# NivekNey/polars-matmul

Measured on AMD Instinct MI355X. Metric: cosine top-k queries/sec, higher is better.
Workload: dtype f32

## Files before the change

polars-matmul_amd/csrc/pmm_kernels.hip:

```cpp
#include "pmm_device.h"

#include <algorithm>

#include <hip/hip_runtime.h>
#include <math.h>
#include <stdint.h>

#include <type_traits>

namespace pmm {

hipError_t launch_norms_f32(const float *a, int64_t rows, int64_t d, int64_t ld, int squared,
                            float *out, float *inv, hipStream_t s) {
  if (rows <= 0) return hipSuccess;
  const int64_t threads = rows * 8;
  const unsigned grid = (unsigned)((threads + 255) / 256);
  norms_kernel<float><<<grid, 256, 0, s>>>(a, rows, d, ld, squared, out, inv);
  return hipGetLastError();
}
hipError_t launch_norms_pair_f32(const float *q, int64_t m, int64_t ldq, float *qout, const float *c,
                                 int64_t n, int64_t ldc, float *cout, float *cinv, int64_t d, int squared,
                                 hipStream_t s, void *zero, size_t zero_bytes) {
  const unsigned gq = (unsigned)((m * 8 + 255) / 256), gc = (unsigned)((n * 8 + 255) / 256);
  if (zero_bytes % 16 != 0 || ((uintptr_t)zero & 15)) return hipErrorInvalidValue;
// ... 1695 lines not shown
  auto lds = [&](int nsp) { return lds_base + RQ * nsp * 8; };
  if (a.ns <= 256) prologue_kernel<4, METRIC, LDSK><<<grid, 256, lds(256), s>>>(a);
  else if (a.ns <= 512) prologue_kernel<8, METRIC, LDSK><<<grid, 256, lds(512), s>>>(a);
  else prologue_kernel<16, METRIC, LDSK><<<grid, 256, lds(1024), s>>>(a);
  return hipGetLastError();
}
template <int METRIC>
static hipError_t launch_prologue_t(const PrologueArgs &a, unsigned grid, hipStream_t s) {
  return a.lds_seed ? launch_prologue_t2<METRIC, 1>(a, grid, s) : launch_prologue_t2<METRIC, 0>(a, grid, s);
}

#ifndef PMM_SEED_MFMA_DEFAULT
#define PMM_SEED_MFMA_DEFAULT 1
#endif
hipError_t launch_seeded_prologue(const float *q, int64_t ldq, int m, const float *c, int64_t ldc, int64_t n,
                                  int d, int dp, int ns, int k, int metric, float *qn, float *cn, bool corpus_norms,
                                  unsigned long long *gthr, void *z0, size_t z0_bytes, void *z1, size_t z1_bytes,
                                  hipStream_t s) {
  if (m <= 0) return hipSuccess;
  if (ns > kSeedMaxNs || k > ns || ns > n || dp % 32 != 0 || dp > kSeedDotsMaxD || d > dp || ldq % 4 != 0 ||
      ldc % 4 != 0 || (((uintptr_t)q | (uintptr_t)c | (uintptr_t)z0 | (uintptr_t)z1) & 15) || z0_bytes % 16 ||
      z1_bytes % 16)
    return hipErrorInvalidValue;
  PrologueArgs a{};
  a.q = q;
  a.ldq = ldq;
  a.m = m;
  a.c = c;
  a.ldc = ldc;
  a.n = n;
  a.d = d;
  a.dp = dp;
  a.ns = ns;
  a.k = k;
  a.squared = metric == kMetricEuclidean;
  a.qn = qn;
  a.cn = cn;
  a.cinv = cn + n;
  a.gthr = gthr;
  a.z0 = (uint4 *)z0;
  a.z1 = (uint4 *)z1;
  a.z0n = (int64_t)(z0_bytes / 16);
  a.z1n = (int64_t)(z1_bytes / 16);
#ifdef PMM_LAB
  a.ablate = getenv("PMM_PROLOGUE_ABLATE") ? atoi(getenv("PMM_PROLOGUE_ABLATE")) : 0;
#endif
  const char *le = getenv("PMM_SEED_LDS");
  a.lds_seed = (ns <= 256 && dp <= seedk::kLdsMaxDp && le && atoi(le) == 1) ? 1 : 0;
  const bool xf = metric != kMetricDot;
  const char *me = getenv("PMM_SEED_MFMA");
  const bool mfma_ok = ns == seedm::NSM && dp <= seedm::kMaxDp && !a.lds_seed && n >= seedm::NSM;
  a.mfma_seed = (mfma_ok && (me ? atoi(me) != 0 : PMM_SEED_MFMA_DEFAULT != 0)) ? 1 : 0;
  if (a.mfma_seed) {
    a.sblocks = (unsigned)((m + seedm::RM - 1) / seedm::RM);
    constexpr int T = seedm::NT;
    a.qblocks = xf ? (unsigned)((m * 8 + T - 1) / T) : 0u;
    a.cblocks = (xf && corpus_norms) ? (unsigned)((n * 8 + T - 1) / T) : 0u;
    a.zblocks = (unsigned)std::max<int64_t>(1, std::min<int64_t>((a.z0n + a.z1n + T - 1) / T, 16));
    const unsigned grid = a.sblocks + a.qblocks + a.cblocks + a.zblocks;
    if (metric == kMetricCosine) return launch_prologue_mfma_t<kMetricCosine>(a, grid, s);
    if (metric == kMetricDot) return launch_prologue_mfma_t<kMetricDot>(a, grid, s);
    return launch_prologue_mfma_t<kMetricEuclidean>(a, grid, s);
  }
  a.sblocks = (unsigned)((m + seedk::RQ - 1) / seedk::RQ);
  unsigned grid;
  if (a.lds_seed) {
    a.qblocks = 0u;
    grid = std::max<unsigned>(a.sblocks, (xf && corpus_norms) ? (unsigned)((n + 63) / 64) : 1u);
    a.cper = (n + grid - 1) / grid;
    a.cblocks = (xf && corpus_norms) ? 1u : 0u;
    a.zblocks = 0u;
  } else {
    a.qblocks = xf ? (unsigned)((m * 8 + 255) / 256) : 0u;
    a.cblocks = (xf && corpus_norms) ? (unsigned)((n * 8 + 255) / 256) : 0u;
    a.zblocks = (unsigned)std::max<int64_t>(1, std::min<int64_t>((a.z0n + a.z1n + 255) / 256, 64));
    grid = a.sblocks + a.qblocks + a.cblocks + a.zblocks;
  }
  if (metric == kMetricCosine) return launch_prologue_t<kMetricCosine>(a, grid, s);
  if (metric == kMetricDot) return launch_prologue_t<kMetricDot>(a, grid, s);
  return launch_prologue_t<kMetricEuclidean>(a, grid, s);
}

constexpr int kMergeRankMaxRows = 16384;
hipError_t launch_merge(const MergeArgs &a0, int loader, hipStream_t s) {
  if (a0.M <= 0) return hipSuccess;
  MergeArgs a = a0;
  static const int rank_env = getenv("PMM_MERGE_RANK") ? atoi(getenv("PMM_MERGE_RANK")) : -1;
  a.no_rank = rank_env == 0 || (rank_env < 0 && a.M > kMergeRankMaxRows);
  a.flags = getenv("PMM_MERGE_FLAGS") ? atoi(getenv("PMM_MERGE_FLAGS"))
                                     : (kMergeReverse | kMergePipelined | kMergeSplitRow);
  const bool sorted = loader == 1 && a.sorted && a.S <= 64 && a.k_out <= 256 && a.P <= 512 &&
                      !(getenv("PMM_MERGE_SORTED") && atoi(getenv("PMM_MERGE_SORTED")) == 0);
  static const int kp = getenv("PMM_KWAY_P") ? atoi(getenv("PMM_KWAY_P")) : 24;
  if (sorted && a.S >= 5 && a.S <= 8 && a.k_out <= 8 * (kp == 32 ? 32 : 24) &&
      !(getenv("PMM_MERGE_KWAY") && atoi(getenv("PMM_MERGE_KWAY")) == 0) &&
      (size_t)MPN(a.P) * 8 <= (size_t)64 * (kp == 32 ? 32 : 24) * 8) {
    static const int wpb = getenv("PMM_KWAY_WPB") ? atoi(getenv("PMM_KWAY_WPB")) : 4;
    const int rows_per_block = 8 * wpb;
    const unsigned grid = (unsigned)((a.M + rows_per_block - 1) / rows_per_block);
    if (kp != 32) {
      if (wpb == 4) (void)hipFuncSetAttribute((const void *)kway_merge_kernel<24>, hipFuncAttributeMaxDynamicSharedMemorySize, 160 * 1024);
      kway_merge_kernel<24><<<grid, 64 * wpb, (size_t)wpb * 64 * 24 * 8, s>>>(a);
    } else {
      if (wpb == 4) (void)hipFuncSetAttribute((const void *)kway_merge_kernel<32>, hipFuncAttributeMaxDynamicSharedMemorySize, 160 * 1024);
      kway_merge_kernel<32><<<grid, 64 * wpb, (size_t)wpb * 64 * 32 * 8, s>>>(a);
    }
    return hipGetLastError();
  }
  if (!(a.S >= 8 && a.k_out <= 64 && a.P <= 512 && !a.no_rank && a.ablate == 0) || sorted) a.flags &= ~kMergeSplitRow;
  const bool split = (a.flags & kMergeSplitRow) != 0;
  int wpb = (int)(65536 / merge_lds_bytes_per_wave(a.P));
  wpb = split ? 4 : (wpb < 1 ? 1 : (wpb > 4 ? 4 : wpb));
  const size_t lds = (size_t)wpb * merge_lds_bytes_per_wave(a.P) + (split ? 16 : 0);
  const unsigned grid = split ? (unsigned)a.M : (unsigned)((a.M + wpb - 1) / wpb);
  if (lds > 65536) {
    static bool attr_set[2] = {false, false};
    if (!attr_set[loader]) {
      const void *fn = loader == 0 ? (const void *)merge_kernel<0, false> : (const void *)merge_kernel<1, false>;
      hipError_t e = hipFuncSetAttribute(fn, hipFuncAttributeMaxDynamicSharedMemorySize, 160 * 1024);
      if (e != hipSuccess) return e;
      attr_set[loader] = true;
    }
  }
  if (sorted) {
    merge_kernel<1, false, true><<<grid, wpb * 64, lds, s>>>(a);
  } else if (split) {
    if (loader == 0) merge_kernel<0, true><<<grid, wpb * 64, lds, s>>>(a);
    else merge_kernel<1, true><<<grid, wpb * 64, lds, s>>>(a);
  } else {
    if (loader == 0) merge_kernel<0, false><<<grid, wpb * 64, lds, s>>>(a);
    else merge_kernel<1, false><<<grid, wpb * 64, lds, s>>>(a);
  }
  return hipGetLastError();
}


template <typename T>
__device__ __forceinline__ u64 score_key(T v, int metric);
template <>
__device__ __forceinline__ u64 score_key<float>(float v, int metric) {
  return (u64)okey32(metric == kMetricEuclidean ? -v : v);
}
template <>
__device__ __forceinline__ u64 score_key<double>(double v, int metric) {
  return okey64(metric == kMetricEuclidean ? -v : v);
}
template <typename T>
__device__ __forceinline__ T key_score(u64 k, int metric);
template <>
__device__ __forceinline__ float key_score<float>(u64 k, int metric) {
  const float v = dekey32((uint32_t)k);
  return metric == kMetricEuclidean ? 0.0f - v : v;
}
template <>
__device__ __forceinline__ double key_score<double>(u64 k, int metric) {
  const double v = dekey64(k);
  return metric == kMetricEuclidean ? 0.0 - v : v;
}

__device__ int ent_compact(Ent *scr, int cnt, int k, int P, Ent *Tv, bool *tfull, int lane) {
  for (int i = cnt + lane; i < P; i += 64) scr[i] = Ent{0ull, 0xFFFFFFFFu, 0u};
  wave_sync();
  wave_sort_desc_ent(scr, P, lane);
  if (cnt >= k) {
    *Tv = scr[k - 1];
    *tfull = true;
    cnt = k;
  }
  wave_sync();
  return cnt;
}

template <typename T>
__global__ __launch_bounds__(256) void rowselect_kernel(RowSelArgs a) {
  extern __shared__ __attribute__((aligned(16))) char smem[];
  const int lane = threadIdx.x & 63, wid = threadIdx.x >> 6;
  const int wpb = blockDim.x >> 6;
  const int row = blockIdx.x * wpb + wid;
  if (row >= a.rows) return;
  Ent *scr = (Ent *)smem + (size_t)wid * a.P;
  const T *src = (const T *)a.scores + (int64_t)row * a.lds;
  Ent Tv{0ull, 0xFFFFFFFFu, 0u};
  bool tfull = false;
  int cnt = 0;
  for (int i0 = 0; i0 < a.N; i0 += 64) {
    const int j = i0 + lane;
    Ent x{0ull, 0xFFFFFFFFu, 0u};
    bool keep = false;
    if (j < a.N) {
      x.key = score_key<T>(src[j], a.metric);
      x.idx = (uint32_t)j;
      keep = !tfull || ent_better(x, Tv);
    }
    const u64 m = __ballot(keep);
    const int pos = cnt + lanes_below(m);
    if (keep) scr[pos] = x;
    cnt += __popcll(m);
    if (cnt > a.P - 64) {
      wave_sync();
      cnt = ent_compact(scr, cnt, a.k, a.P, &Tv, &tfull, lane);
    }
  }
  wave_sync();
  const int P2 = min(a.P, next_pow2_dev(cnt));
  for (int i = cnt + lane; i < P2; i += 64) scr[i] = Ent{0ull, 0xFFFFFFFFu, 0u};
  wave_sync();
  wave_sort_desc_ent(scr, P2, lane);
  T *os = (T *)a.out_score;
  for (int j = lane; j < a.k; j += 64) {
    const Ent x = scr[j];
    a.out_idx[(int64_t)row * a.k + j] = x.idx + a.index_base;
    os[(int64_t)row * a.k + j] = key_score<T>(x.key, a.metric);
  }
}

hipError_t launch_rowselect(const RowSelArgs &a, hipStream_t s) {
  if (a.rows <= 0) return hipSuccess;
  const size_t per_wave = (size_t)a.P * sizeof(Ent);
  int wpb = (int)(65536 / per_wave);
  wpb = wpb < 1 ? 1 : (wpb > 4 ? 4 : wpb);
  const size_t lds = (size_t)wpb * per_wave;
  const unsigned grid = (unsigned)((a.rows + wpb - 1) / wpb);
  if (a.is_f64) rowselect_kernel<double><<<grid, wpb * 64, lds, s>>>(a);
  else rowselect_kernel<float><<<grid, wpb * 64, lds, s>>>(a);
  return hipGetLastError();
}

template <typename T>
__global__ void rowsort_build(const T *__restrict__ scores, int64_t lds, int rows, int N, int P2,
                              int metric, Ent *__restrict__ keys) {
  const int64_t t = (int64_t)blockIdx.x * blockDim.x + threadIdx.x;
  if (t >= (int64_t)rows * P2) return;
  const int r = (int)(t / P2), j = (int)(t % P2);
  Ent e{0ull, 0xFFFFFFFFu, 0u};
  if (j < N) {
    e.key = score_key<T>(scores[(int64_t)r * lds + j], metric);
    e.idx = (uint32_t)j;
  }
  keys[t] = e;
}
__global__ void rowsort_step(Ent *keys, int rows, int P2, int size, int stride) {
  const int64_t t = (int64_t)blockIdx.x * blockDim.x + threadIdx.x;
  const int64_t half = (int64_t)P2 >> 1;
  if (t >= (int64_t)rows * half) return;
  const int r = (int)(t / half), i = (int)(t % half);
  const int x0 = ((i & ~(stride - 1)) << 1) | (i & (stride - 1));
  const int x1 = x0 + stride;
  Ent *base = keys + (int64_t)r * P2;
  const Ent a = base[x0], b = base[x1];
  const bool desc = (x0 & size) == 0;
  if (desc ? ent_better(b, a) : ent_better(a, b)) {
    base[x0] = b;
    base[x1] = a;
  }
}
template <typename T>
__global__ void rowsort_extract(const Ent *__restrict__ keys, int rows, int P2, int k, int metric,
                                uint32_t index_base, uint32_t *__restrict__ out_idx,
                                T *__restrict__ out_score) {
  const int64_t t = (int64_t)blockIdx.x * blockDim.x + threadIdx.x;
  if (t >= (int64_t)rows * k) return;
  const int r = (int)(t / k), j = (int)(t % k);
  const Ent e = keys[(int64_t)r * P2 + j];
  out_idx[t] = e.idx + index_base;
  out_score[t] = key_score<T>(e.key, metric);
}

hipError_t launch_rowsort_global(const void *scores, int64_t lds, int rows, int N, int is_f64,
                                 int metric, void *keys_ws, int P2, int k, uint32_t index_base,
                                 uint32_t *out_idx, void *out_score, hipStream_t s) {
  if (rows <= 0) return hipSuccess;
  Ent *keys = (Ent *)keys_ws;
  const int64_t tot = (int64_t)rows * P2;
  const unsigned gb = (unsigned)((tot + 255) / 256);
  if (is_f64) rowsort_build<double><<<gb, 256, 0, s>>>((const double *)scores, lds, rows, N, P2, metric, keys);
  else rowsort_build<float><<<gb, 256, 0, s>>>((const float *)scores, lds, rows, N, P2, metric, keys);
  const unsigned gs = (unsigned)((tot / 2 + 255) / 256);
  for (int size = 2; size <= P2; size <<= 1)
    for (int stride = size >> 1; stride > 0; stride >>= 1)
      rowsort_step<<<gs, 256, 0, s>>>(keys, rows, P2, size, stride);
  const int64_t tk = (int64_t)rows * k;
  const unsigned ge = (unsigned)((tk + 255) / 256);
  if (is_f64) rowsort_extract<double><<<ge, 256, 0, s>>>(keys, rows, P2, k, metric, index_base, out_idx, (double *)out_score);
  else rowsort_extract<float><<<ge, 256, 0, s>>>(keys, rows, P2, k, metric, index_base, out_idx, (float *)out_score);
  return hipGetLastError();
}

__global__ __launch_bounds__(256) void screen_prep_kernel(const float *__restrict__ rel,
                                                          const unsigned *__restrict__ scal, int m, int dp,
                                                          float *__restrict__ eps, u64 *gthr, int seeded) {
  const int row = (int)(blockIdx.x * blockDim.x + threadIdx.x);
  if (row >= m) return;
  const float e = screen_eps(rel[row], __uint_as_float(scal[0]), dp);
  eps[row] = e;
  if (seeded) gthr[row] = screen_lower(gthr[row], e);
}
hipError_t launch_screen_prep(const float *rel, const unsigned *scal, int m, int dp, float *eps,
                              unsigned long long *gthr, int seeded, hipStream_t s) {
  if (m <= 0) return hipSuccess;
  screen_prep_kernel<<<(unsigned)((m + 255) / 256), 256, 0, s>>>(rel, scal, m, dp, eps, gthr, seeded);
  return hipGetLastError();
}

constexpr int kRescoreList = 512;

template <typename F>
__device__ __forceinline__ void rescore_each_entry(const ScreenFinishArgs &a, u64 *base, const unsigned *segs,
                                                   int nseg, F &&f) {
  const int tid = threadIdx.x, nt = blockDim.x;
  for (int t = 0; t < nseg; t++) {
    const unsigned e = segs[t];
    const int n = (int)(e & 1023u);
    u64 *seg = base + (int64_t)(e >> 10) * a.capg;
    for (int i0 = tid; i0 < n; i0 += 4 * nt) {
      u64 x[4];
#pragma unroll
      for (int j = 0; j < 4; j++) x[j] = i0 + j * nt < n ? seg[i0 + j * nt] : 0ull;
#pragma unroll
      for (int j = 0; j < 4; j++)
        if (i0 + j * nt < n) f(seg + i0 + j * nt, x[j]);
    }
  }
}

__global__ __launch_bounds__(256, 8) void screen_rescore_kernel(ScreenFinishArgs a) {
  extern __shared__ __attribute__((aligned(16))) char smem[];
  __shared__ __attribute__((aligned(16))) unsigned hist[256];
  __shared__ unsigned list[kRescoreList];
  __shared__ unsigned res[4], ln, emin;
  float *qs = (float *)smem;
  unsigned *segs = (unsigned *)(qs + a.dp);
  const int tid = threadIdx.x, nt = blockDim.x;
  const int row = (int)blockIdx.x;
  const float *qr = a.q + (int64_t)row * a.ldq;
  for (int i = 4 * tid; i < a.dp; i += 4 * nt) *(f32x4 *)(qs + i) = *(const f32x4 *)(qr + i);
  for (int i = tid; i < 256; i += nt) hist[i] = 0u;
  if (tid == 0) emin = ~0u, ln = 0u;
  __syncthreads();
  for (int s = tid; s < a.S; s += nt) {
    const unsigned n = min(a.cnt[(int64_t)row * a.S + s], (unsigned)a.capg);
    if (n) segs[atomicAdd(&ln, 1u)] = ((unsigned)s << 10) | n;
  }
  __syncthreads();
  const int nseg = (int)ln;
  const float qv = a.qn[row];
  const float eps = a.eps[row];
  const u64 T = screen_lower(a.gthr[row], eps);
  const u64 T1 = T ? T : 1ull;
  u64 *base = a.cand + (int64_t)row * a.S * a.capg;

  auto live = [&](u64 x) __attribute__((always_inline)) -> bool {
    return x >= T1 && ~(uint32_t)x < (uint32_t)a.N;
  };
  u64 P = 0ull;
  unsigned n_r = 0u, need = (unsigned)a.k;
  for (int shift = 56; shift >= 0; shift -= 8) {
    rescore_each_entry(a, base, segs, nseg, [&](u64 *, u64 x) __attribute__((always_inline)) {
      if (live(x) && (shift == 56 || ((x ^ P) >> (shift + 8)) == 0ull))
        atomicAdd(&hist[(unsigned)(x >> shift) & 255u], 1u);
    });
    __syncthreads();
    if (tid < 64) {
      const uint4 h = ((const uint4 *)hist)[tid];
      ((uint4 *)hist)[tid] = make_uint4(0u, 0u, 0u, 0u);
      const unsigned own = h.x + h.y + h.z + h.w;
      unsigned suf = own;
#pragma unroll
      for (int o = 1; o < 64; o <<= 1) {
        const unsigned t = __shfl_down(suf, o);
        if (tid + o < 64) suf += t;
      }
      if (tid == 0) {
        res[0] = res[1] = res[2] = 0u;
        if (shift == 56) res[3] = suf;
      }
      unsigned above = suf - own;
      if (above < need && suf >= need) {
        unsigned b = 3u, in_bin = h.w;
        if (above + in_bin < need) above += in_bin, in_bin = h.z, b = 2u;
        if (above + in_bin < need) above += in_bin, in_bin = h.y, b = 1u;
        if (above + in_bin < need) above += in_bin, in_bin = h.x, b = 0u;
        res[0] = 4u * (unsigned)tid + b;
        res[1] = need - above;
        res[2] = in_bin;
      }
    }
    __syncthreads();
    P |= (u64)res[0] << shift;
    need = res[1];
    if (shift == 56) n_r = res[3];
    if (res[2] == need) break;
  }
  const int max_rounds = (int)(((int64_t)a.S * a.capg + kRescoreList - 1) / kRescoreList) + 1;
  unsigned done = 0u;
  for (int ph = n_r > (unsigned)a.k ? 1 : 2; ph <= 2; ph++) {
    const bool last = ph == 2;
    u64 thr = P;
    if (last) {
      __syncthreads();
      const u64 E = screen_lower((u64)emin << 32, eps);
      thr = E > T1 ? E : T1;
    }
    for (int r = 0; r < max_rounds; r++) {
      __syncthreads();
      if (tid == 0) ln = 0u;
      __syncthreads();
      rescore_each_entry(a, base, segs, nseg, [&](u64 *p, u64 x) __attribute__((always_inline)) {
        if (x == 0ull) return;
        const uint32_t lw = (uint32_t)x;
        if (!(lw & 0x80000000u)) return;
        if (x < thr || !live(x)) {
          if (last) *p = 0ull;
          return;
        }
        const unsigned pos = atomicAdd(&ln, 1u);
        if (pos < (unsigned)kRescoreList) list[pos] = (unsigned)(p - base);
      });
      __syncthreads();
      const unsigned n = ln;
      const bool more = n > (unsigned)kRescoreList;
      const int cnt = more ? kRescoreList : (int)n;
      for (int t = tid; t < cnt; t += nt) {
        u64 *p = base + list[t];
        const uint32_t col = ~(uint32_t)*p;
        const float *cr = a.c + (int64_t)col * a.ldc;
        float acc = 0.0f;
        for (int k0 = 0; k0 < a.dp; k0 += 32) {
          f32x4 v[8];
#pragma unroll
          for (int j = 0; j < 8; j++) v[j] = *(const f32x4 *)(cr + k0 + 4 * j);
#pragma unroll
          for (int j = 0; j < 8; j++) {
            const f32x4 q4 = *(const f32x4 *)(qs + k0 + 4 * j);
            acc = fmaf(q4[0], v[j][0], acc);
            acc = fmaf(q4[1], v[j][1], acc);
            acc = fmaf(q4[2], v[j][2], acc);
            acc = fmaf(q4[3], v[j][3], acc);
          }
        }
        const uint32_t key = okey32(exact_score<kMetricCosine>(acc, qv, a.cn[col]));
        if (!last) atomicMin(&emin, key);
        *p = ((u64)key << 32) | (u64)col;
        done++;
      }
      if (!more) break;
    }
  }
  __syncthreads();
  rescore_each_entry(a, base, segs, nseg, [&](u64 *p, u64 x) __attribute__((always_inline)) {
    if (x != 0ull && !((uint32_t)x & 0x80000000u)) *p = (x & 0xFFFFFFFF00000000ull) | (u64)(~(uint32_t)x);
  });
  if (a.stat) {
    __syncthreads();
    if (tid == 0) ln = 0u;
    __syncthreads();
    atomicAdd(&ln, done);
    __syncthreads();
    if (tid == 0) {
      atomicAdd(a.stat, ln);
      atomicMax(a.stat + 1, ln);
      atomicAdd(a.stat + 2, n_r);
    }
  }
}
hipError_t launch_screen_rescore(const ScreenFinishArgs &a, hipStream_t s) {
  if (a.M <= 0) return hipSuccess;
  if (a.dp % 32 != 0 || a.dp > 4096 || a.ldq % 4 != 0 || a.ldc % 4 != 0 || a.ldq < a.dp || a.ldc < a.dp ||
      (((uintptr_t)a.q | (uintptr_t)a.c) & 15) || a.k < 1 || a.k > kRescoreList || a.capg > 1023 ||
      ((int64_t)a.dp + a.S) * 4 > 64 * 1024)
    return hipErrorInvalidValue;
  int nt = 64;
  if (const char *e = getenv("PMM_RESCORE_BLOCK")) {
    const int v = atoi(e);
    if (v == 64 || v == 128 || v == 256) nt = v;
  }
  screen_rescore_kernel<<<(unsigned)a.M, nt, ((size_t)a.dp + a.S) * 4, s>>>(a);
  return hipGetLastError();
}

__device__ __forceinline__ bool is_pos_zero(float v) { return __float_as_uint(v) == 0u; }
__device__ __forceinline__ bool is_pos_zero(double v) { return __double_as_longlong(v) == 0ll; }
__device__ __forceinline__ float fma_chain_step(float a, float b, float c) { return fmaf(a, b, c); }
__device__ __forceinline__ double fma_chain_step(double a, double b, double c) { return __fma_rn(a, b, c); }
__device__ __forceinline__ float cosine_of(float dot, float qv, float cv) {
  return exact_score<kMetricCosine>(dot, qv, cv);
}
__device__ __forceinline__ double cosine_of(double dot, double qv, double cv) {
  return exact_score_f64<kMetricCosine>(dot, qv, cv);
}
template <typename T>
__global__ __launch_bounds__(256) void zero_sign_kernel(const T *__restrict__ q, int64_t ldq,
                                                        const T *__restrict__ c, int64_t ldc,
                                                        const T *__restrict__ qn, const T *__restrict__ cn,
                                                        int m, int64_t n, int d, int k, int metric,
                                                        uint32_t index_base, const uint32_t *__restrict__ out_idx,
                                                        T *__restrict__ out_score,
                                                        const uint32_t *__restrict__ qrow) {
  const int64_t t = (int64_t)blockIdx.x * blockDim.x + threadIdx.x;
  if (t >= (int64_t)m * k) return;
  if (!is_pos_zero(out_score[t])) return;
  const uint32_t id = out_idx ? out_idx[t] : (uint32_t)(t % k) + index_base;
  if (id == 0xFFFFFFFFu) return;
  const int64_t col = (int64_t)(uint32_t)(id - index_base);
  if (col >= n) return;
  const int64_t row = qrow ? (int64_t)qrow[t / k] : t / k;
  const T *qr = q + row * ldq, *cr = c + col * ldc;
  T acc = (T)0;
  for (int i = 0; i < d; i++) acc = fma_chain_step(qr[i], cr[i], acc);
  const T sc = metric == kMetricDot ? acc : cosine_of(acc, qn[row], cn[col]);
  if (sc == (T)0) out_score[t] = sc;
}
hipError_t launch_zero_sign_f32(const float *q, int64_t ldq, const float *c, int64_t ldc, const float *qn,
                                const float *cn, int m, int64_t n, int d, int k, int metric, uint32_t index_base,
                                const uint32_t *out_idx, float *out_score, hipStream_t s, const uint32_t *qrow) {
  if (m <= 0 || k <= 0 || metric == kMetricEuclidean) return hipSuccess;
  zero_sign_kernel<float><<<(unsigned)(((int64_t)m * k + 255) / 256), 256, 0, s>>>(
      q, ldq, c, ldc, qn, cn, m, n, d, k, metric, index_base, out_idx, out_score, qrow);
  return hipGetLastError();
}
hipError_t launch_zero_sign_f64(const double *q, int64_t ldq, const double *c, int64_t ldc, const double *qn,
                                const double *cn, int m, int64_t n, int d, int k, int metric, uint32_t index_base,
                                const uint32_t *out_idx, double *out_score, hipStream_t s) {
  if (m <= 0 || k <= 0 || metric == kMetricEuclidean) return hipSuccess;
  zero_sign_kernel<double><<<(unsigned)(((int64_t)m * k + 255) / 256), 256, 0, s>>>(
      q, ldq, c, ldc, qn, cn, m, n, d, k, metric, index_base, out_idx, out_score, nullptr);
  return hipGetLastError();
}

__global__ __launch_bounds__(256) void zero_sign_lists_kernel(const uint32_t *__restrict__ in_idx,
                                                              const float *__restrict__ in_score, int lists,
                                                              int k_in, int64_t row_stride, int64_t list_stride,
                                                              int m, int k, const uint32_t *__restrict__ out_idx,
                                                              float *__restrict__ out_score) {
  const int64_t t = (int64_t)blockIdx.x * blockDim.x + threadIdx.x;
  if (t >= (int64_t)m * k) return;
  if (__float_as_uint(out_score[t]) != 0u) return;
  const uint32_t id = out_idx[t];
  if (id == 0xFFFFFFFFu) return;
  const int64_t row = t / k;
  for (int g = 0; g < lists; g++) {
    const int64_t base = (int64_t)g * list_stride + row * row_stride;
    for (int j = 0; j < k_in; j++) {
      if (in_idx[base + j] != id) continue;
      const float sc = in_score[base + j];
      if (sc == 0.0f) out_score[t] = sc;
      return;
    }
  }
}
hipError_t launch_zero_sign_lists(const uint32_t *in_idx, const float *in_score, int lists, int k_in,
                                  int64_t row_stride, int64_t list_stride, int m, int k, const uint32_t *out_idx,
                                  float *out_score, hipStream_t s) {
  if (m <= 0 || k <= 0 || lists <= 0) return hipSuccess;
  zero_sign_lists_kernel<<<(unsigned)(((int64_t)m * k + 255) / 256), 256, 0, s>>>(
      in_idx, in_score, lists, k_in, row_stride, list_stride, m, k, out_idx, out_score);
  return hipGetLastError();
}

__global__ __launch_bounds__(256) void screen_collect_kernel(const unsigned *__restrict__ ovf,
                                                             const unsigned *__restrict__ bad, int m,
                                                             unsigned *count, int *__restrict__ rows) {
  const int row = (int)(blockIdx.x * blockDim.x + threadIdx.x);
  if (row < m && (ovf[row] | bad[row])) {
    rows[atomicAdd(count, 1u)] = row;
    if (ovf[row]) atomicAdd(count + 1, 1u);
  }
}
hipError_t launch_screen_collect(const unsigned *ovf, const unsigned *bad, int m, unsigned *count, int *rows,
                                 hipStream_t s) {
  if (m <= 0) return hipSuccess;
  screen_collect_kernel<<<(unsigned)((m + 255) / 256), 256, 0, s>>>(ovf, bad, m, count, rows);
  return hipGetLastError();
}

__global__ __launch_bounds__(256) void gather_rows_kernel(const uint4 *__restrict__ src, int64_t ld,
                                                          const int *__restrict__ rows, int r, int units,
                                                          uint4 *__restrict__ dst) {
  const int64_t t = (int64_t)blockIdx.x * blockDim.x + threadIdx.x;
  if (t >= (int64_t)r * units) return;
  const int i = (int)(t / units), c = (int)(t - (int64_t)i * units);
  dst[t] = src[(int64_t)rows[i] * ld + c];
}
hipError_t launch_gather_rows(const void *src, int64_t ld_units, const int *rows, int r, int units, void *dst,
                              hipStream_t s) {
  if (r <= 0 || units <= 0) return hipSuccess;
  gather_rows_kernel<<<(unsigned)(((int64_t)r * units + 255) / 256), 256, 0, s>>>((const uint4 *)src, ld_units, rows,
                                                                                  r, units, (uint4 *)dst);
  return hipGetLastError();
}
__global__ __launch_bounds__(256) void scatter_lists_kernel(const uint32_t *__restrict__ oi,
                                                            const float *__restrict__ os,
                                                            const int *__restrict__ rows, int r, int k,
                                                            uint32_t *__restrict__ out_idx,
                                                            float *__restrict__ out_score) {
  const int64_t t = (int64_t)blockIdx.x * blockDim.x + threadIdx.x;
  if (t >= (int64_t)r * k) return;
  const int i = (int)(t / k), j = (int)(t - (int64_t)i * k);
  out_idx[(int64_t)rows[i] * k + j] = oi[t];
  out_score[(int64_t)rows[i] * k + j] = os[t];
}
hipError_t launch_scatter_lists(const uint32_t *oi, const float *os, const int *rows, int r, int k,
                                uint32_t *out_idx, float *out_score, hipStream_t s) {
  if (r <= 0) return hipSuccess;
  scatter_lists_kernel<<<(unsigned)(((int64_t)r * k + 255) / 256), 256, 0, s>>>(oi, os, rows, r, k, out_idx,
                                                                               out_score);
  return hipGetLastError();
}

}
```

Measured before the change: 605,700.

## Stage rescore candidate rows through LDS tile with coalesced loads and prefetch ring

The exact-rescore loop now has the 64-lane block cooperatively load 16 candidate rows per step into an LDS tile. Each lane issues two 16-byte loads per 32-float chunk, with a two-step prefetch ring, replacing the old scheme where each thread streamed a whole row alone. The list size is halved, the histogram shares storage with the lists, and the column is cached in LDS. The final restore pass is skipped in favour of touching only the remembered phase-1 offsets when no overflow happened. The cost is two block barriers per chunk, and only 16 of 64 lanes do the FMA work.

```diff
diff --git a/polars-matmul_amd/csrc/pmm_kernels.hip b/polars-matmul_amd/csrc/pmm_kernels.hip
--- a/polars-matmul_amd/csrc/pmm_kernels.hip
+++ b/polars-matmul_amd/csrc/pmm_kernels.hip
@@ -2021,7 +2021,15 @@
   return hipGetLastError();
 }
 
-constexpr int kRescoreList = 512;
+constexpr int kRescoreList = 256;
+constexpr int kRescoreThreads = 64;
+constexpr int kRescoreRows = 16;
+constexpr int kRescoreChunk = 32;
+constexpr int kRescoreStride = kRescoreChunk + 4;
+constexpr int kRescoreAhead = 2;
+constexpr int kRescoreP1 = (kRescoreList + kRescoreThreads - 1) / kRescoreThreads;
+static_assert(kRescoreRows * (kRescoreChunk / 4) == 2 * kRescoreThreads, "two 16-byte loads per lane and step");
+static_assert(2 * kRescoreList >= 256, "the selection's histogram lies in the lists' storage");
 
 template <typename F>
 __device__ __forceinline__ void rescore_each_entry(const ScreenFinishArgs &a, u64 *base, const unsigned *segs,
@@ -2042,14 +2050,19 @@
   }
 }
 
-__global__ __launch_bounds__(256, 8) void screen_rescore_kernel(ScreenFinishArgs a) {
+struct RescoreLoads {
+  f32x4 v[2];
+};
+
+__global__ __launch_bounds__(kRescoreThreads, 5) void screen_rescore_kernel(ScreenFinishArgs a) {
   extern __shared__ __attribute__((aligned(16))) char smem[];
-  __shared__ __attribute__((aligned(16))) unsigned hist[256];
-  __shared__ unsigned list[kRescoreList];
+  __shared__ __attribute__((aligned(16))) unsigned lbuf[2 * kRescoreList];
+  __shared__ __attribute__((aligned(16))) float tile[kRescoreRows * kRescoreStride];
   __shared__ unsigned res[4], ln, emin;
+  unsigned *hist = lbuf, *loff = lbuf, *lcol = lbuf + kRescoreList;
   float *qs = (float *)smem;
   unsigned *segs = (unsigned *)(qs + a.dp);
-  const int tid = threadIdx.x, nt = blockDim.x;
+  const int tid = threadIdx.x, nt = kRescoreThreads;
   const int row = (int)blockIdx.x;
   const float *qr = a.q + (int64_t)row * a.ldq;
   for (int i = 4 * tid; i < a.dp; i += 4 * nt) *(f32x4 *)(qs + i) = *(const f32x4 *)(qr + i);
@@ -2079,7 +2092,7 @@
         atomicAdd(&hist[(unsigned)(x >> shift) & 255u], 1u);
     });
     __syncthreads();
-    if (tid < 64) {
+    {
       const uint4 h = ((const uint4 *)hist)[tid];
       ((uint4 *)hist)[tid] = make_uint4(0u, 0u, 0u, 0u);
       const unsigned own = h.x + h.y + h.z + h.w;
@@ -2111,6 +2124,12 @@
     if (res[2] == need) break;
   }
   const int max_rounds = (int)(((int64_t)a.S * a.capg + kRescoreList - 1) / kRescoreList) + 1;
+  const int nchunk = a.dp / kRescoreChunk;
+  const int lrow = tid >> 3, piece = (tid & 7) * 4;
+  unsigned p1off[kRescoreP1];
+#pragma unroll
+  for (int j = 0; j < kRescoreP1; j++) p1off[j] = ~0u;
+  bool several = false;
   unsigned done = 0u;
   for (int ph = n_r > (unsigned)a.k ? 1 : 2; ph <= 2; ph++) {
     const bool last = ph == 2;
@@ -2133,42 +2152,99 @@
           return;
         }
         const unsigned pos = atomicAdd(&ln, 1u);
-        if (pos < (unsigned)kRescoreList) list[pos] = (unsigned)(p - base);
+        if (pos < (unsigned)kRescoreList) loff[pos] = (unsigned)(p - base), lcol[pos] = ~lw;
       });
       __syncthreads();
       const unsigned n = ln;
       const bool more = n > (unsigned)kRescoreList;
       const int cnt = more ? kRescoreList : (int)n;
-      for (int t = tid; t < cnt; t += nt) {
-        u64 *p = base + list[t];
-        const uint32_t col = ~(uint32_t)*p;
-        const float *cr = a.c + (int64_t)col * a.ldc;
-        float acc = 0.0f;
-        for (int k0 = 0; k0 < a.dp; k0 += 32) {
-          f32x4 v[8];
-#pragma unroll
-          for (int j = 0; j < 8; j++) v[j] = *(const f32x4 *)(cr + k0 + 4 * j);
-#pragma unroll
-          for (int j = 0; j < 8; j++) {
-            const f32x4 q4 = *(const f32x4 *)(qs + k0 + 4 * j);
-            acc = fmaf(q4[0], v[j][0], acc);
-            acc = fmaf(q4[1], v[j][1], acc);
-            acc = fmaf(q4[2], v[j][2], acc);
-            acc = fmaf(q4[3], v[j][3], acc);
+      several = several || more;
+      const bool marked = !last || more;
+      if (!last) {
+#pragma unroll
+        for (int j = 0; j < kRescoreP1; j++) {
+          const int t = tid + j * kRescoreThreads;
+          p1off[j] = t < cnt ? loff[t] : ~0u;
+        }
+      }
+      const int nsteps = ((cnt + kRescoreRows - 1) / kRescoreRows) * nchunk;
+      int lg = 0, lc = 0;
+      const float *rp0 = a.c, *rp1 = a.c;
+      bool lv0 = false, lv1 = false;
+      auto issue = [&](RescoreLoads &x, int s) __attribute__((always_inline)) {
+        if (s >= nsteps) return;
+        if (lc == 0) {
+          const int t0 = lg + lrow, t1 = t0 + 8;
+          lv0 = t0 < cnt;
+          lv1 = t1 < cnt;
+          if (lv0) rp0 = a.c + (int64_t)lcol[t0] * a.ldc + piece;
+          if (lv1) rp1 = a.c + (int64_t)lcol[t1] * a.ldc + piece;
+        }
+        if (lv0) x.v[0] = *(const f32x4 *)(rp0 + lc * kRescoreChunk);
+        if (lv1) x.v[1] = *(const f32x4 *)(rp1 + lc * kRescoreChunk);
+        if (++lc == nchunk) lc = 0, lg += kRescoreRows;
+      };
+      int sg = 0, sc = 0;
+      float acc = 0.0f, cnv = 0.0f;
+      auto score = [&](const RescoreLoads &x) __attribute__((always_inline)) {
+        if (sg + lrow < cnt) *(f32x4 *)(tile + lrow * kRescoreStride + piece) = x.v[0];
+        if (sg + lrow + 8 < cnt) *(f32x4 *)(tile + (lrow + 8) * kRescoreStride + piece) = x.v[1];
+        __syncthreads();
+        const int t = sg + tid;
+        if (tid < kRescoreRows && t < cnt) {
+          if (sc == 0) acc = 0.0f, cnv = a.cn[lcol[t]];
+          const float *tr = tile + tid * kRescoreStride;
+          const float *qk = qs + sc * kRescoreChunk;
+#pragma unroll
+          for (int j = 0; j < kRescoreChunk / 4; j++) {
+            const f32x4 v = *(const f32x4 *)(tr + 4 * j);
+            const f32x4 q4 = *(const f32x4 *)(qk + 4 * j);
+            acc = fmaf(q4[0], v[0], acc);
+            acc = fmaf(q4[1], v[1], acc);
+            acc = fmaf(q4[2], v[2], acc);
+            acc = fmaf(q4[3], v[3], acc);
+          }
+          if (sc == nchunk - 1) {
+            const uint32_t col = lcol[t];
+            const uint32_t key = okey32(exact_score<kMetricCosine>(acc, qv, cnv));
+            if (!last) atomicMin(&emin, key);
+            base[loff[t]] = ((u64)key << 32) | (u64)(marked ? col : ~col);
+            done++;
           }
         }
-        const uint32_t key = okey32(exact_score<kMetricCosine>(acc, qv, a.cn[col]));
-        if (!last) atomicMin(&emin, key);
-        *p = ((u64)key << 32) | (u64)col;
-        done++;
+        __syncthreads();
+        if (++sc == nchunk) sc = 0, sg += kRescoreRows;
+      };
+      RescoreLoads ring[kRescoreAhead] = {};
+#pragma unroll
+      for (int j = 0; j < kRescoreAhead; j++) issue(ring[j], j);
+      for (int s = 0; s < nsteps; s += kRescoreAhead) {
+#pragma unroll
+        for (int j = 0; j < kRescoreAhead; j++) {
+          if (s + j < nsteps) {
+            const RescoreLoads cur = ring[j];
+            issue(ring[j], s + j + kRescoreAhead);
+            score(cur);
+          }
+        }
       }
       if (!more) break;
     }
   }
   __syncthreads();
-  rescore_each_entry(a, base, segs, nseg, [&](u64 *p, u64 x) __attribute__((always_inline)) {
+  auto restore = [&](u64 *p, u64 x) __attribute__((always_inline)) {
     if (x != 0ull && !((uint32_t)x & 0x80000000u)) *p = (x & 0xFFFFFFFF00000000ull) | (u64)(~(uint32_t)x);
-  });
+  };
+  if (several) {
+    rescore_each_entry(a, base, segs, nseg, restore);
+  } else {
+    u64 x[kRescoreP1];
+#pragma unroll
+    for (int j = 0; j < kRescoreP1; j++) x[j] = p1off[j] != ~0u ? base[p1off[j]] : 0ull;
+#pragma unroll
+    for (int j = 0; j < kRescoreP1; j++)
+      if (p1off[j] != ~0u) restore(base + p1off[j], x[j]);
+  }
   if (a.stat) {
     __syncthreads();
     if (tid == 0) ln = 0u;
@@ -2184,16 +2260,11 @@
 }
 hipError_t launch_screen_rescore(const ScreenFinishArgs &a, hipStream_t s) {
   if (a.M <= 0) return hipSuccess;
-  if (a.dp % 32 != 0 || a.dp > 4096 || a.ldq % 4 != 0 || a.ldc % 4 != 0 || a.ldq < a.dp || a.ldc < a.dp ||
-      (((uintptr_t)a.q | (uintptr_t)a.c) & 15) || a.k < 1 || a.k > kRescoreList || a.capg > 1023 ||
+  if (a.dp % kRescoreChunk != 0 || a.dp > 4096 || a.ldq % 4 != 0 || a.ldc % 4 != 0 || a.ldq < a.dp ||
+      a.ldc < a.dp || (((uintptr_t)a.q | (uintptr_t)a.c) & 15) || a.k < 1 || a.k > kRescoreList || a.capg > 1023 ||
       ((int64_t)a.dp + a.S) * 4 > 64 * 1024)
     return hipErrorInvalidValue;
-  int nt = 64;
-  if (const char *e = getenv("PMM_RESCORE_BLOCK")) {
-    const int v = atoi(e);
-    if (v == 64 || v == 128 || v == 256) nt = v;
-  }
-  screen_rescore_kernel<<<(unsigned)a.M, nt, ((size_t)a.dp + a.S) * 4, s>>>(a);
+  screen_rescore_kernel<<<(unsigned)a.M, kRescoreThreads, ((size_t)a.dp + a.S) * 4, s>>>(a);
   return hipGetLastError();
 }
 
```

New measurement: 650,100, median of 6. +7.3%, better.
